# huang-yh/SelfOcc

Hardware: AMD Instinct MI355X
Metric: rendered rays/sec (6-cam 450x800, 128 samples/ray) (higher is better)
Workload: dtype f32; 1 GPU; BASELINE configs[1]: 6 cams x 450x800 rays, 128 samples/ray, volume 200x200x16; volume_channels=1, feat_storage=f32, preheat_steps=150

## Files before the change

### selfocc_amd/csrc/render_fwd.hip

```cpp
#include "so_device.h"
#include "sh_device.h"
#include "ray_device.h"

template <int NF, bool BF16>
int so_render_fwd_samples(const so_render_args &a, hipStream_t st);
template <int NB>
int so_render_sh_samples(const so_render_args &a, hipStream_t st);

namespace {

SO_DEVFN RayGeom so_pixel_ray(const so_render_args &a, int cam, int ix, int iy) {
    typedef const __attribute__((address_space(4))) float *so_const_fptr;
    const so_const_fptr M = (so_const_fptr)(a.img2lidar + cam * 16);
    float u = (float)ix * a.sx + a.ox;
    float v = (float)iy * a.sy + a.oy;
    RayGeom g;
    g.ox = M[3]; g.oy = M[7]; g.oz = M[11];
    float dx = (M[0] * u + M[1] * v) + M[2];
    float dy = (M[4] * u + M[5] * v) + M[6];
    float dz = (M[8] * u + M[9] * v) + M[10];
    g.dn = sqrtf((dx * dx + dy * dy) + dz * dz);
    g.dx = dx / g.dn; g.dy = dy / g.dn; g.dz = dz / g.dn;
    return g;
}
// ... 345 lines not shown
#pragma unroll
        for (int kk = 0; kk < 8; ++kk) {
            const int h = h0 + (kk >> 2), w = w0 + ((kk >> 1) & 1), d = d0 + (kk & 1);
            const bool in = ((unsigned)h < (unsigned)H) && ((unsigned)w < (unsigned)W) && ((unsigned)d < (unsigned)D);
            const int li = ((min(max(h, 0), H - 1) - hmin) * 4 + (min(max(w, 0), W - 1) - wmin)) * 4 +
                           (min(max(d, 0), D - 1) - dmin);
            const float wgt = in ? wk[kk] : 0.0f;
            const float4 *p = (const float4 *)(lds + li * ST);
#pragma unroll
            for (int q = 0; q < NF / 4; ++q) {
                const float4 t = p[q];
                so_fma4_bcast(f[4 * q + 0], f[4 * q + 1], f[4 * q + 2], f[4 * q + 3], t.x, t.y,
                              t.z, t.w, wgt);
            }
        }
    }
    __builtin_amdgcn_fence(__ATOMIC_RELEASE, "wavefront");
    __builtin_amdgcn_wave_barrier();
}

SO_DEVFN so_render_args so_reload_args() {
    typedef const __attribute__((address_space(4))) uint32_t *so_kernarg_ptr;
    so_kernarg_ptr ka = (so_kernarg_ptr)__builtin_amdgcn_kernarg_segment_ptr();
    asm volatile("" : "+s"(ka));
    so_render_args ac;
    static_assert(sizeof(ac) % 4 == 0, "so_render_args is dword-sized");
#pragma unroll
    for (unsigned k = 0; k < sizeof(ac) / 4; ++k) ((uint32_t *)&ac)[k] = ka[k];
    return ac;
}

template <int NF>
struct FastStep {
    float fh, fw, fd, fi;
    int h0, w0, d0;
    unsigned cell;
    bool all_interior;
    float v[8];
    unsigned code;
    bool boxed, pref;
    int hmin, wmin, dmin;
    so_f4v blk[NF >= 4 ? NF / 4 : 1];
};

template <int NF, bool BF16, bool STAGED = false, bool FACE_SAFE = false, class GeomFn>
SO_DEVFN void so_march_fast(const so_render_args &a, int ray, GeomFn geom, bool store = true,
                             float *lds = nullptr, int lane = 0, float *sem_lds = nullptr) {
    constexpr int NSEM = NF > 4 ? NF - 3 : 0;
    constexpr bool SEM_LDS = STAGED && NSEM >= 16;
    const RayGeom g = geom(a);
    const int H = a.map.h.tot_len, W = a.map.w.tot_len, D = a.map.d.tot_len;
    const int S = a.n_samples;
    float tnear, tfar;
    so_collide(a, g, tnear, tfar);
    const float dt = (tfar - tnear) / (float)S;
    const float inv_dn = 1.0f / g.dn;

    const AxisK kh = so_axis_affine(a.map.h), kw = so_axis_affine(a.map.w), kd = so_axis_affine(a.map.d);
    const float t_off = (a.sample_pos == SO_SAMPLE_AT_START) ? tnear : tnear + 0.5f * dt;
    const float Gdh = g.dy * kh.k1, Gdw = g.dx * kw.k1, Gdd = g.dz * kd.k1;
    const float G0h = fmaf(g.oy, kh.k1, kh.k0) + Gdh * t_off;
    const float G0w = fmaf(g.ox, kw.k1, kw.k0) + Gdw * t_off;
    const float G0d = fmaf(g.oz, kd.k1, kd.k0) + Gdd * t_off;
    const float s2 = so_inv_s(a) * 1.44269504088896341f;
    const float hdt = 0.5f * dt;
    const float hdt_s2 = hdt * s2;

    float T = 1.0f, acc = 0.0f, dsum = 0.0f;
    float rgb[3] = {0.0f, 0.0f, 0.0f};
    float sem[(NSEM > 0 && !SEM_LDS) ? NSEM : 1];
    if constexpr (SEM_LDS) {
#pragma unroll
        for (int k = 0; k < NSEM; ++k) sem_lds[k * 256] = 0.0f;
    } else {
#pragma unroll
        for (int k = 0; k < NSEM; ++k) sem[k] = 0.0f;
    }
    float best_w = -1.0f, best_t = 0.0f;
    const float *__restrict__ vol = a.sdf_vol;
    const __amdgpu_buffer_rsrc_t rs = so_make_rsrc(vol, (size_t)H * W * D * 4);
    const unsigned sD = (unsigned)D * 4u, sWD = (unsigned)W * D * 4u;
    const bool use_brick = a.sdf_brick != nullptr;
    const unsigned n_cells = (unsigned)(H * W * D);
    const __amdgpu_buffer_rsrc_t rb = so_make_rsrc(a.sdf_brick, use_brick ? (size_t)n_cells * 33 : 0);
    const unsigned lane_vox = (unsigned)(((lane >> 4) * W + ((lane >> 2) & 3)) * D + (lane & 3));
    const __amdgpu_buffer_rsrc_t rf = so_make_rsrc(a.feat_vol, NF > 0 ? (size_t)H * W * D * NF * (BF16 ? 2 : 4) : 0);
    constexpr bool CAN_SKIP = NF == 0;
    const bool use_skip = CAN_SKIP && use_brick && !(a.flags & SO_FLAG_NO_SKIP);
    const int rcode = use_skip ? max((int)ceilf(dt / so_skip_unit(a.aabb, S)), 1) : 0x7fffffff;
    const int maxdim = max(H, max(W, D));
    const float face_m = 3.0f * 1.1920929e-7f * (float)(1u << (32 - __builtin_clz((unsigned)maxdim)));

    constexpr bool FACE_LATE = FACE_SAFE && NF == 0;
    auto near_face = [&](float fh, float fw, float fd) __attribute__((always_inline)) {
        return fmaxf(fmaxf(fabsf(fh - 0.5f), fabsf(fw - 0.5f)), fabsf(fd - 0.5f)) > 0.5f - face_m;
    };
    auto canon_cell = [&](const int i) __attribute__((always_inline)) {
        if constexpr (NF < 8) {
            const float b0 = so_bin(i, S);
            const float t_start = b0 * tfar + (1.0f - b0) * tnear;
            float px, py, pz;
            if (a.sample_pos == SO_SAMPLE_AT_START) {
                px = g.ox + g.dx * t_start; py = g.oy + g.dy * t_start; pz = g.oz + g.dz * t_start;
            } else {
                const float b1 = so_bin(i + 1, S);
                const float tt = t_start + (b1 * tfar + (1.0f - b1) * tnear);
                px = g.ox + (g.dx * tt) / 2.0f; py = g.oy + (g.dy * tt) / 2.0f; pz = g.oz + (g.dz * tt) / 2.0f;
            }
            return so_locate(a.map, px, py, pz);
        } else {
            const so_render_args ac = so_reload_args();
            const RayGeom gc = geom(ac);
            float tn, tf;
            so_collide(ac, gc, tn, tf);
            const float t_start = so_edge(ac, ray, i, tn, tf);
            float px, py, pz;
            if (ac.sample_pos == SO_SAMPLE_AT_START) {
                px = gc.ox + gc.dx * t_start; py = gc.oy + gc.dy * t_start; pz = gc.oz + gc.dz * t_start;
            } else {
                const float tt = t_start + so_edge(ac, ray, i + 1, tn, tf);
                px = gc.ox + (gc.dx * tt) / 2.0f; py = gc.oy + (gc.dy * tt) / 2.0f; pz = gc.oz + (gc.dz * tt) / 2.0f;
            }
            return so_locate(ac.map, px, py, pz);
        }
    };

    constexpr bool PIPE = NF < 8;
    auto fetch = [&](const int i, FastStep<NF> &st) __attribute__((always_inline)) {
        st.fi = (float)i;
        const float step = st.fi * dt;
        const float gh = fmaf(Gdh, step, G0h), gw = fmaf(Gdw, step, G0w), gd = fmaf(Gdd, step, G0d);
        st.fh = __builtin_amdgcn_fractf(gh); st.fw = __builtin_amdgcn_fractf(gw); st.fd = __builtin_amdgcn_fractf(gd);
        int h0 = so_floor_i(gh), w0 = so_floor_i(gw), d0 = so_floor_i(gd);
        if constexpr (FACE_SAFE && !FACE_LATE) {
            if (__any(near_face(st.fh, st.fw, st.fd))) {
                if (near_face(st.fh, st.fw, st.fd)) {
                    const so_cell c = canon_cell(i);
                    h0 = c.h0; w0 = c.w0; d0 = c.d0;
                    st.fh = c.fh1; st.fw = c.fw1; st.fd = c.fd1;
                }
            }
        }
        st.h0 = h0; st.w0 = w0; st.d0 = d0;
        const bool interior = ((unsigned)h0 < (unsigned)(H - 1)) & ((unsigned)w0 < (unsigned)(W - 1)) &
                              ((unsigned)d0 < (unsigned)(D - 1));
        st.all_interior = so_all(interior);
        st.cell = so_cell_index(h0, w0, d0, W, D);
        st.code = 0u;
        if (st.all_interior) {
            if (use_brick) {
                const unsigned vo = st.cell * 32u;
                const so_f4v lo = so_bload4(rb, vo, 0u), hi = so_bload4(rb, vo + 16u, 0u);
                if constexpr (CAN_SKIP) {
                    if (use_skip) st.code = __builtin_amdgcn_raw_buffer_load_b8(rb, st.cell, n_cells * 32u, 0);
                }
                st.v[0] = lo.x; st.v[4] = lo.y; st.v[1] = lo.z; st.v[5] = lo.w;
                st.v[2] = hi.x; st.v[6] = hi.y; st.v[3] = hi.z; st.v[7] = hi.w;
            } else {
                const unsigned vo = st.cell * 4u;
                const so_f2v p00 = so_bload2(rs, vo, 0u), p01 = so_bload2(rs, vo, sD);
                const so_f2v p10 = so_bload2(rs, vo, sWD), p11 = so_bload2(rs, vo, sWD + sD);
                st.v[0] = p00.x; st.v[1] = p00.y; st.v[2] = p01.x; st.v[3] = p01.y;
                st.v[4] = p10.x; st.v[5] = p10.y; st.v[6] = p11.x; st.v[7] = p11.y;
            }
        } else {
            const int d0c = min(max(d0, 0), D - 2);
            const bool dlo_in = (unsigned)d0 < (unsigned)D, dhi_in = (unsigned)(d0 + 1) < (unsigned)D;
            const bool lo_first = (d0 == d0c), hi_first = (d0 + 1 == d0c);
#pragma unroll
            for (int q = 0; q < 4; ++q) {
                const int h = h0 + (q >> 1), w = w0 + (q & 1);
                const bool in = ((unsigned)h < (unsigned)H) && ((unsigned)w < (unsigned)W);
                const int hc = min(max(h, 0), H - 1), wc = min(max(w, 0), W - 1);
                const so_f2u pr = *(const so_f2u *)(vol + ((hc * W + wc) * D + d0c));
                const float lo = lo_first ? pr.x : pr.y, hi = hi_first ? pr.x : pr.y;
                st.v[2 * q] = (in && dlo_in) ? lo : 0.0f;
                st.v[2 * q + 1] = (in && dhi_in) ? hi : 0.0f;
            }
        }
        st.boxed = false; st.pref = false;
        if constexpr (STAGED) {
            st.boxed = so_stage_box(h0, w0, d0, H, W, D, st.hmin, st.wmin, st.dmin);
            if (PIPE && st.boxed && st.hmin + 3 < H && st.wmin + 3 < W && st.dmin + 3 < D) {
                const unsigned vo = ((unsigned)((st.hmin * W + st.wmin) * D + st.dmin) + lane_vox) * (NF * 4u);
#pragma unroll
                for (int q = 0; q < NF / 4; ++q) st.blk[q] = so_bload4(rf, vo + q * 16u, 0u);
                st.pref = true;
            }
        }
    };

    auto consume = [&](const int i, FastStep<NF> &st) __attribute__((always_inline)) {
        const float fi = st.fi;
        const float *v = st.v;
        float w, sdf = 0.0f, gvw = 0.0f, gvd = 0.0f, gvh = 0.0f;
        bool skip = false;
        if constexpr (CAN_SKIP) skip = so_all((int)st.code >= rcode);
        if (skip) {
            w = kAlphaFree * T;
            T = T * ((1.0f - kAlphaFree) + 1e-7f);
        } else {
            if constexpr (FACE_LATE) {
                if (__any(near_face(st.fh, st.fw, st.fd))) {
                    if (near_face(st.fh, st.fw, st.fd)) {
                        const so_cell c = canon_cell(i);
                        if (c.h0 != st.h0 || c.w0 != st.w0 || c.d0 != st.d0) {
                            so_gather_sdf(vol, H, W, D, c, st.v);
                            st.fh = c.fh1; st.fw = c.fw1; st.fd = c.fd1;
                            st.h0 = c.h0; st.w0 = c.w0; st.d0 = c.d0;
                        }
                    }
                }
            }
            const float fh = st.fh, fw = st.fw, fd = st.fd;
            const float dd0 = v[1] - v[0], dd1 = v[3] - v[2], dd2 = v[5] - v[4], dd3 = v[7] - v[6];
            const float c0 = fmaf(fd, dd0, v[0]), c1 = fmaf(fd, dd1, v[2]);
            const float c2 = fmaf(fd, dd2, v[4]), c3 = fmaf(fd, dd3, v[6]);
            const float dw0 = c1 - c0, dw1 = c3 - c2;
            const float b0 = fmaf(fw, dw0, c0), b1 = fmaf(fw, dw1, c2);
            const float dh0 = b1 - b0;
            sdf = fmaf(fh, dh0, b0);
            gvw = fmaf(fh, dw1 - dw0, dw0);
            const float e0 = fmaf(fw, dd1 - dd0, dd0), e1 = fmaf(fw, dd3 - dd2, dd2);
            gvd = fmaf(fh, e1 - e0, e0);
            gvh = dh0;

            const float cosv = fmaf(gvd, Gdd, fmaf(gvw, Gdw, gvh * Gdh));
            const float alpha = so_alpha_fast(sdf * s2, fminf(cosv, 0.0f) * hdt_s2);
            w = alpha * T;
            T = T * ((1.0f - alpha) + 1e-7f);
        }

        const float t_mid = fmaf(fi, dt, tnear + hdt);
        acc = acc + w;
        dsum = fmaf(w, t_mid, dsum);
        if (w > best_w) { best_w = w; best_t = t_mid; }

// ... 21 lines not shown
                else so_gather_feat<NF, BF16>(a.feat_vol, H, W, D, c, wk, f);
            }
#pragma unroll
            for (int k = 0; k < 3; ++k) {
                float col = fmaxf(fmaf(0.28209479177387814f, f[k], 0.5f), 0.0f);
                rgb[k] = fmaf(w, col, rgb[k]);
            }
            if constexpr (NSEM > 0) {
                float m = f[3];
#pragma unroll
                for (int k = 1; k < NSEM; ++k) m = fmaxf(m, f[3 + k]);
                float e[NSEM], den = 0.0f;
#pragma unroll
                for (int k = 0; k < NSEM; ++k) {
                    e[k] = so_fast_exp2((f[3 + k] - m) * 1.44269504088896341f);
                    den = den + e[k];
                }
                const float wd = w * so_fast_rcp(den);
                if constexpr (SEM_LDS) {
#pragma unroll
                    for (int k = 0; k < NSEM; ++k) sem_lds[k * 256] = fmaf(wd, e[k], sem_lds[k * 256]);
                } else {
#pragma unroll
                    for (int k = 0; k < NSEM; ++k) sem[k] = fmaf(wd, e[k], sem[k]);
                }
            }
        }
    };

    if constexpr (PIPE) {
        FastStep<NF> A, B;
        fetch(0, A);
        for (int i = 0;;) {
            if (i + 1 < S) fetch(i + 1, B);
            consume(i, A);
            if (++i >= S) break;
            if (so_all(T < 1e-10f)) break;
            if (i + 1 < S) fetch(i + 1, A);
            consume(i, B);
            if (++i >= S) break;
            if (so_all(T < 1e-10f)) break;
        }
    } else {
        for (int i = 0; i < S; ++i) {
            FastStep<NF> A;
            fetch(i, A);
            consume(i, A);
            if (so_all(T < 1e-10f)) break;
        }
    }

    const float eps32 = 1.1920928955078125e-07f;
    if (dt * inv_dn < eps32) best_t = tnear + hdt;
    if (!store) return;
    float depth = dsum * so_fast_rcp(acc + 1e-10f);
    if (a.flags & SO_FLAG_DEPTH_DIV_NORM) depth = depth * inv_dn;
    if (a.depth) a.depth[ray] = depth;
    if (a.acc) a.acc[ray] = acc;
    if (a.max_depth) a.max_depth[ray] = best_t * inv_dn;
    if (a.nears) a.nears[ray] = tnear;
    if (a.fars) a.fars[ray] = tfar;
    if constexpr (NF > 0) {
        if (a.rgb) {
#pragma unroll
            for (int k = 0; k < 3; ++k) {
                float bg = 0.0f;
                if (a.bkgd_mode == SO_BKGD_CONST) bg = a.bkgd[k];
                else if (a.bkgd_mode == SO_BKGD_PER_RAY) bg = a.bkgd_rays[3 * (size_t)ray + k];
                float r = rgb[k];
                if (a.bkgd_mode != SO_BKGD_NONE) r = r + bg * (1.0f - acc);
                if (a.flags & SO_FLAG_CLAMP_RGB) r = fminf(fmaxf(r, 0.0f), 1.0f);
                a.rgb[3 * (size_t)ray + k] = r;
            }
        }
        if constexpr (NSEM > 0) {
            if (a.sem) {
#pragma unroll
                for (int k = 0; k < NSEM; ++k) a.sem[(size_t)ray * NSEM + k] = SEM_LDS ? sem_lds[k * 256] : sem[k];
            }
        }
    }
}

struct AheadStep {
    float gh, gw, gd, fi;
    int h0, w0, d0;
    unsigned cell, code;
    bool all_interior;
};

template <bool FACE_SAFE, class GeomFn>
SO_DEVFN void so_march_fast_ahead(const so_render_args &a, int ray, GeomFn geom) {
    const int H = a.map.h.tot_len, W = a.map.w.tot_len, D = a.map.d.tot_len;
    const int S = a.n_samples;
    const RayGeom g = geom(a);
    float tnear, tfar;
    so_collide(a, g, tnear, tfar);
    const float dt = (tfar - tnear) / (float)S;
    const float inv_dn = 1.0f / g.dn;
    const AxisK kh = so_axis_affine(a.map.h), kw = so_axis_affine(a.map.w), kd = so_axis_affine(a.map.d);
    const float t_off = (a.sample_pos == SO_SAMPLE_AT_START) ? tnear : tnear + 0.5f * dt;
    const float Gdh = g.dy * kh.k1, Gdw = g.dx * kw.k1, Gdd = g.dz * kd.k1;
    const float G0h = fmaf(g.oy, kh.k1, kh.k0) + Gdh * t_off;
    const float G0w = fmaf(g.ox, kw.k1, kw.k0) + Gdw * t_off;
    const float G0d = fmaf(g.oz, kd.k1, kd.k0) + Gdd * t_off;
    const float s2 = so_inv_s(a) * 1.44269504088896341f;
    const float hdt = 0.5f * dt, hdt_s2 = hdt * s2;
    const float *__restrict__ vol = a.sdf_vol;
    const unsigned n_cells = (unsigned)(H * W * D);
    const __amdgpu_buffer_rsrc_t rb = so_make_rsrc(a.sdf_brick, (size_t)n_cells * 33);
    const __amdgpu_buffer_rsrc_t rs = so_make_rsrc(vol, (size_t)n_cells * 4);
    const int rcode = max((int)ceilf(dt / so_skip_unit(a.aabb, S)), 1);
    const int maxdim = max(H, max(W, D));
    const float face_m = 3.0f * 1.1920929e-7f * (float)(1u << (32 - __builtin_clz((unsigned)maxdim)));

    float T = 1.0f, acc = 0.0f, dsum = 0.0f, best_w = -1.0f, best_t = 0.0f;

    auto locate = [&](const int i, AheadStep &st) __attribute__((always_inline)) {
        st.fi = (float)i;
        const float step = st.fi * dt;
        const float gh = fmaf(Gdh, step, G0h), gw = fmaf(Gdw, step, G0w), gd = fmaf(Gdd, step, G0d);
        st.gh = gh; st.gw = gw; st.gd = gd;
        const int h0 = so_floor_i(gh), w0 = so_floor_i(gw), d0 = so_floor_i(gd);
        st.h0 = h0; st.w0 = w0; st.d0 = d0;
        st.all_interior = so_all3((unsigned)h0 < (unsigned)(H - 1), (unsigned)w0 < (unsigned)(W - 1),
                                  (unsigned)d0 < (unsigned)(D - 1));
        st.cell = so_cell_index(h0, w0, d0, W, D);
        st.code = 0u;
        if (st.all_interior) st.code = __builtin_amdgcn_raw_buffer_load_b8(rb, st.cell, n_cells * 32u, 0);
    };
    auto near_face = [&](float fh, float fw, float fd) __attribute__((always_inline)) {
        return fmaxf(fmaxf(fabsf(fh - 0.5f), fabsf(fw - 0.5f)), fabsf(fd - 0.5f)) > 0.5f - face_m;
    };
    auto canon_cell = [&](const int i) __attribute__((always_inline)) {
        const RayGeom gc = geom(so_reload_args());
        __builtin_amdgcn_sched_barrier(0);
        float px, py, pz;
        {
            const so_render_args ac = so_reload_args();
            const int n = ac.n_samples;
            const float b0 = so_bin(i, n);
            const float t_start = b0 * tfar + (1.0f - b0) * tnear;
            if (ac.sample_pos == SO_SAMPLE_AT_START) {
                px = gc.ox + gc.dx * t_start; py = gc.oy + gc.dy * t_start; pz = gc.oz + gc.dz * t_start;
            } else {
                const float b1 = so_bin(i + 1, n);
                const float tt = t_start + (b1 * tfar + (1.0f - b1) * tnear);
                px = gc.ox + (gc.dx * tt) / 2.0f; py = gc.oy + (gc.dy * tt) / 2.0f; pz = gc.oz + (gc.dz * tt) / 2.0f;
            }
        }
        __builtin_amdgcn_sched_barrier(0);
        float slope;
        const float gh = so_grid_coord(so_axis_m2g(so_reload_args().map.h, py, slope), so_reload_args().map.h.tot_len);
        __builtin_amdgcn_sched_barrier(0);
        const float gw = so_grid_coord(so_axis_m2g(so_reload_args().map.w, px, slope), so_reload_args().map.w.tot_len);
        __builtin_amdgcn_sched_barrier(0);
        const float gd = so_grid_coord(so_axis_m2g(so_reload_args().map.d, pz, slope), so_reload_args().map.d.tot_len);
        return so_cell_of(gh, gw, gd);
    };

    auto step = [&](const int i, AheadStep &cur, AheadStep &nxt) __attribute__((always_inline)) {
        const bool skip = cur.all_interior && so_all((int)cur.code >= rcode);
        if (i + 1 < S) locate(i + 1, nxt);
        float w;
        if (skip) {
            w = kAlphaFree * T;
            T = T * ((1.0f - kAlphaFree) + 1e-7f);
        } else {
            float fh = __builtin_amdgcn_fractf(cur.gh), fw = __builtin_amdgcn_fractf(cur.gw), fd = __builtin_amdgcn_fractf(cur.gd);
            so_f32x2 p0, p1, p2, p3;
            auto gather = [&](int h0, int w0, int d0) __attribute__((always_inline)) {
                float v[8];
                so_gather_sdf_buf(rs, H, W, D, h0, w0, d0, v);
                p0 = so_f32x2{v[0], v[4]}; p1 = so_f32x2{v[1], v[5]}; p2 = so_f32x2{v[2], v[6]}; p3 = so_f32x2{v[3], v[7]};
            };
            bool loaded = false;
            if constexpr (FACE_SAFE) {
                if (__any(near_face(fh, fw, fd))) {
                    int h0 = cur.h0, w0 = cur.w0, d0 = cur.d0;
                    bool moved = false;
                    if (near_face(fh, fw, fd)) {
                        const so_cell c = canon_cell(i);
                        if (c.h0 != h0 || c.w0 != w0 || c.d0 != d0) {
                            h0 = c.h0; w0 = c.w0; d0 = c.d0;
                            fh = c.fh1; fw = c.fw1; fd = c.fd1;
                            moved = true;
                        }
                    }
                    if (__any(moved)) { gather(h0, w0, d0); loaded = true; }
                }
            }
            if (!loaded) {
                if (cur.all_interior) {
                    {
                        const so_f4v lo = so_bload4(rb, cur.cell * 32u, 0u), hi = so_bload4(rb, cur.cell * 32u + 16u, 0u);
                        p0 = lo.xy; p1 = lo.zw; p2 = hi.xy; p3 = hi.zw;
                    }
                } else {
                    gather(cur.h0, cur.w0, cur.d0);
                }
            }
            float sdf, dh0, gvw, gvd;
            so_trilerp_fast_pk(p0, p1, p2, p3, fh, fw, fd, sdf, dh0, gvw, gvd);
            const float cosv = fmaf(gvd, Gdd, fmaf(gvw, Gdw, dh0 * Gdh));
            const float alpha = so_alpha_fast(sdf * s2, fminf(cosv, 0.0f) * hdt_s2);
            w = alpha * T;
            T = T * ((1.0f - alpha) + 1e-7f);
        }
        const float t_mid = fmaf(cur.fi, dt, tnear + hdt);
        acc = acc + w;
        dsum = fmaf(w, t_mid, dsum);
        if (w > best_w) { best_w = w; best_t = t_mid; }
    };

    {
        AheadStep A, B;
        locate(0, A);
        for (int i = 0;;) {
            step(i, A, B);
            if (++i >= S) break;
            if (so_all(T < 1e-10f)) break;
            step(i, B, A);
            if (++i >= S) break;
            if (so_all(T < 1e-10f)) break;
        }
    }

    const float eps32 = 1.1920928955078125e-07f;
    if (dt * inv_dn < eps32) best_t = tnear + hdt;
    float depth = dsum * so_fast_rcp(acc + 1e-10f);
    if (a.flags & SO_FLAG_DEPTH_DIV_NORM) depth = depth * inv_dn;
    if (a.depth) a.depth[ray] = depth;
    if (a.acc) a.acc[ray] = acc;
    if (a.max_depth) a.max_depth[ray] = best_t * inv_dn;
    if (a.nears) a.nears[ray] = tnear;
    if (a.fars) a.fars[ray] = tfar;
}

enum class March {
    Canonical,
    Fast,
    FastFaceSafe,
    Skip,
    SkipFaceSafe,
    CanonicalUpscale,
};
constexpr bool so_is_fast(March m) { return m == March::Fast || m == March::FastFaceSafe; }
constexpr bool so_is_skip(March m) { return m == March::Skip || m == March::SkipFaceSafe; }
constexpr bool so_face_safe(March m) { return m == March::FastFaceSafe || m == March::SkipFaceSafe; }
template <int NF, bool BF16>
constexpr bool so_is_staged(March m) { return so_is_fast(m) && !BF16 && NF >= 4; }

template <int NF, bool BF16, March MODE, class GeomFn>
SO_DEVFN void so_march(const so_render_args &a, int ray, GeomFn geom) {
    if constexpr (MODE == March::CanonicalUpscale) {
        so_march_exact<NF, BF16, SO_MAP_UPSCALE>(a, ray, geom(a));
    } else if constexpr (so_is_skip(MODE)) {
        static_assert(NF == 0, "skip marcher: SDF-only launches");
        so_march_fast_ahead<so_face_safe(MODE)>(a, ray, geom);
    } else if constexpr (so_is_fast(MODE)) {
        so_march_fast<NF, BF16, false, so_face_safe(MODE)>(a, ray, geom);
    } else {
        so_march_exact<NF, BF16>(a, ray, geom(a));
    }
}


__global__ __launch_bounds__(256) void sdf_brickify_kernel(const float *__restrict__ vol, float *__restrict__ brick,
                                                           int H, int W, int D, so_render_args a, int with_codes) {
    const int cell = blockIdx.x * blockDim.x + threadIdx.x;
    if (cell >= H * W * D) return;
    const int d = cell % D, w = (cell / D) % W, h = cell / (D * W);
    const int h1 = min(h + 1, H - 1), w1 = min(w + 1, W - 1), d1 = min(d + 1, D - 1);
    const float *r00 = vol + ((size_t)h * W + w) * D, *r01 = vol + ((size_t)h * W + w1) * D;
    const float *r10 = vol + ((size_t)h1 * W + w) * D, *r11 = vol + ((size_t)h1 * W + w1) * D;
    const float v0 = r00[d], v1 = r00[d1], v2 = r01[d], v3 = r01[d1];
    const float v4 = r10[d], v5 = r10[d1], v6 = r11[d], v7 = r11[d1];
    float4 *o = (float4 *)(brick + (size_t)cell * 8);
    o[0] = make_float4(v0, v4, v1, v5);
    o[1] = make_float4(v2, v6, v3, v7);
    uint8_t *codes = (uint8_t *)(brick + (size_t)H * W * D * 8);
    unsigned code = 0u;
    if (with_codes) {
        const float m = fminf(fminf(fminf(v0, v1), fminf(v2, v3)), fminf(fminf(v4, v5), fminf(v6, v7)));
        const float gd = fmaxf(fmaxf(fabsf(v1 - v0), fabsf(v3 - v2)), fmaxf(fabsf(v5 - v4), fabsf(v7 - v6))) *
                         (a.map.d.size0 / a.map.d.range0);
        const float gw = fmaxf(fmaxf(fabsf(v2 - v0), fabsf(v3 - v1)), fmaxf(fabsf(v6 - v4), fabsf(v7 - v5))) *
                         (a.map.w.size0 / a.map.w.range0);
        const float gh = fmaxf(fmaxf(fabsf(v4 - v0), fabsf(v5 - v1)), fmaxf(fabsf(v6 - v2), fabsf(v7 - v3))) *
                         (a.map.h.size0 / a.map.h.range0);
        const float G = sqrtf((gd * gd + gw * gw) + gh * gh) * 1.001f + 1e-20f;
        const float slack = m - kSkipArg / so_inv_s(a);
        if (slack > 0.0f && so_inv_s(a) > 0.0f) {
            const float allow = 2.0f * slack / G / so_skip_unit(a.aabb, a.n_samples);
            code = (unsigned)fminf(floorf(allow * 0.999f), 255.0f);
        }
    }
    codes[cell] = (uint8_t)code;
}

struct TilePixel { int cam, ix, iy, wave, lane; };
SO_DEVFN TilePixel so_tile_pixel(int tiles_x, int tiles_y) {
    const int b = blockIdx.x;
    const int cam = b / (tiles_x * tiles_y);
    const int tb = b - cam * tiles_x * tiles_y;
    const int ty = tb / tiles_x, tx = tb - ty * tiles_x;
    const int wave = threadIdx.x >> 6, lane = threadIdx.x & 63;
    return {cam, tx * 16 + (wave & 1) * 8 + (lane & 7), ty * 16 + (wave >> 1) * 8 + (lane >> 3), wave, lane};
}

template <int NF, bool BF16, March MODE>
__global__ __launch_bounds__(256, (NF >= 8 ? 2 : 1)) void render_fwd_explicit(so_render_args a) {
    int ray = blockIdx.x * blockDim.x + threadIdx.x;
    if (ray >= a.n_rays) return;
    auto geom = [&](const so_render_args &a) __attribute__((always_inline)) { return so_explicit_ray(a, ray); };
    so_march<NF, BF16, MODE>(a, ray, geom);
}

template <int NF, bool BF16, March MODE>
SO_DEVFN void pixgrid_body(const so_render_args &a, int tiles_x, int tiles_y) {
    const TilePixel p = so_tile_pixel(tiles_x, tiles_y);
    const int cam = p.cam, wave = p.wave, lane = p.lane;
    int ix = p.ix, iy = p.iy;
    if constexpr (so_is_staged<NF, BF16>(MODE)) {
        __shared__ __attribute__((aligned(16))) float s_stage[4 * StageGeom<NF>::kWaveDwords];
        const bool real = (ix < a.nx) && (iy < a.ny);
        ix = min(ix, a.nx - 1); iy = min(iy, a.ny - 1);
        int ray = (cam * a.ny + iy) * a.nx + ix;
        auto geom = [&](const so_render_args &a) __attribute__((always_inline)) { return so_pixel_ray(a, cam, ix, iy); };
        constexpr int NSEM_LDS = NF - 3 >= 16 ? NF - 3 : 0;
        __shared__ float s_sem[NSEM_LDS > 0 ? NSEM_LDS * 256 : 1];
        so_march_fast<NF, BF16, true, so_face_safe(MODE)>(a, ray, geom, real, s_stage + wave * StageGeom<NF>::kWaveDwords, lane,
                                                          s_sem + threadIdx.x);
    } else {
        if (ix >= a.nx || iy >= a.ny) return;
        int ray = (cam * a.ny + iy) * a.nx + ix;
        auto geom = [&](const so_render_args &a) __attribute__((always_inline)) { return so_pixel_ray(a, cam, ix, iy); };
        so_march<NF, BF16, MODE>(a, ray, geom);
    }
}

template <int NF, bool BF16, March MODE>
__global__ __launch_bounds__(256, (NF >= 8 ? 2 : 1)) void render_fwd_pixgrid(so_render_args a, int tiles_x, int tiles_y) {
    pixgrid_body<NF, BF16, MODE>(a, tiles_x, tiles_y);
}
template <>
__global__ __launch_bounds__(256, 1) __attribute__((amdgpu_num_sgpr(80))) void render_fwd_pixgrid<0, false, March::Skip>(
    so_render_args a, int tiles_x, int tiles_y) {
    pixgrid_body<0, false, March::Skip>(a, tiles_x, tiles_y);
}
template <>
__global__ __launch_bounds__(256, 1) __attribute__((amdgpu_num_sgpr(80))) void render_fwd_pixgrid<0, false, March::SkipFaceSafe>(
    so_render_args a, int tiles_x, int tiles_y) {
    pixgrid_body<0, false, March::SkipFaceSafe>(a, tiles_x, tiles_y);
}

template <int NF, bool BF16, March MODE>
int launch_fwd(const so_render_args &a, hipStream_t st) {
    if (a.ray_mode == SO_RAYS_EXPLICIT) {
        int blocks = (a.n_rays + 255) / 256;
        hipLaunchKernelGGL((render_fwd_explicit<NF, BF16, MODE>), dim3(blocks), dim3(256), 0, st, a);
    } else {
        int tiles_x = (a.nx + 15) / 16, tiles_y = (a.ny + 15) / 16;
        int blocks = tiles_x * tiles_y * a.n_cams;
        hipLaunchKernelGGL((render_fwd_pixgrid<NF, BF16, MODE>), dim3(blocks), dim3(256), 0, st, a, tiles_x, tiles_y);
    }
    return so_launch_status();
}

template <int NF, bool BF16>
int dispatch_ps(const so_render_args &a, hipStream_t st) {
    bool per_sample = a.weights || a.ts || a.deltas || a.sdf || a.grad;
    if (per_sample) return so_render_fwd_samples<NF, BF16>(a, st);
    if (a.map.kind == SO_MAP_UPSCALE) {
        if constexpr (NF == 24 && BF16) {
            SO_REQUIRE(false, "the 'linear_upscale' mapping is built for n_rgb + n_sem = 0, 3, 8 and float32 24 (got bfloat16 24)");
        } else {
            return launch_fwd<NF, BF16, March::CanonicalUpscale>(a, st);
        }
    }
    bool fast = !(a.flags & SO_FLAG_EXACT) && a.jitter_mode == SO_JITTER_NONE && a.map.kind == SO_MAP_LINEAR &&
                a.map.h.size1 == 0.0f && a.map.w.size1 == 0.0f && a.map.d.size1 == 0.0f &&
                (long long)a.map.h.tot_len * a.map.w.tot_len < (1 << 24) && a.map.d.tot_len < (1 << 24);
    if (fast) {
        if (a.sdf_brick) {
            const int cells = a.map.h.tot_len * a.map.w.tot_len * a.map.d.tot_len;
            const int with_codes = (NF == 0 && !(a.flags & SO_FLAG_NO_SKIP)) ? 1 : 0;
            hipLaunchKernelGGL(sdf_brickify_kernel, dim3((cells + 255) / 256), dim3(256), 0, st, a.sdf_vol, a.sdf_brick,
                               a.map.h.tot_len, a.map.w.tot_len, a.map.d.tot_len, a, with_codes);
        }
        if constexpr (NF == 0) {
            if (a.sdf_brick && !(a.flags & (SO_FLAG_NO_SKIP | SO_FLAG_NO_AHEAD)))
                return (a.flags & SO_FLAG_NO_FACE_SAFE) ? launch_fwd<0, false, March::Skip>(a, st) : launch_fwd<0, false, March::SkipFaceSafe>(a, st);
        }
        if (!(a.flags & SO_FLAG_NO_FACE_SAFE)) return launch_fwd<NF, BF16, March::FastFaceSafe>(a, st);
        return launch_fwd<NF, BF16, March::Fast>(a, st);
    }
    return launch_fwd<NF, BF16, March::Canonical>(a, st);
}

template <int NB, int MK>
__global__ __launch_bounds__(256) void render_sh_explicit(so_render_args a) {
    const int ray = blockIdx.x * blockDim.x + threadIdx.x;
    if (ray >= a.n_rays) return;
    so_march_exact<so_sh_stride(NB), false, MK, NB>(a, ray, so_explicit_ray(a, ray));
}

template <int NB, int MK>
__global__ __launch_bounds__(256) void render_sh_pixgrid(so_render_args a, int tiles_x, int tiles_y) {
    const int b = blockIdx.x;
    const int cam = b / (tiles_x * tiles_y);
    const int tb = b - cam * tiles_x * tiles_y;
    const int ty = tb / tiles_x, tx = tb - ty * tiles_x;
    const int wave = threadIdx.x >> 6, lane = threadIdx.x & 63;
    const int ix = tx * 16 + (wave & 1) * 8 + (lane & 7);
    const int iy = ty * 16 + (wave >> 1) * 8 + (lane >> 3);
    if (ix >= a.nx || iy >= a.ny) return;
    const int ray = (cam * a.ny + iy) * a.nx + ix;
    so_march_exact<so_sh_stride(NB), false, MK, NB>(a, ray, so_pixel_ray(a, cam, ix, iy));
}

template <int NB, int MK>
int launch_sh(const so_render_args &a, hipStream_t st) {
    if (a.ray_mode == SO_RAYS_EXPLICIT) {
        hipLaunchKernelGGL((render_sh_explicit<NB, MK>), dim3((a.n_rays + 255) / 256), dim3(256), 0, st, a);
    } else {
        const int tiles_x = (a.nx + 15) / 16, tiles_y = (a.ny + 15) / 16;
        hipLaunchKernelGGL((render_sh_pixgrid<NB, MK>), dim3(tiles_x * tiles_y * a.n_cams), dim3(256), 0, st, a, tiles_x, tiles_y);
    }
    return so_launch_status();
}

template <int NB>
int dispatch_sh(const so_render_args &a, hipStream_t st) {
    if (a.weights || a.ts || a.deltas || a.sdf || a.grad) return so_render_sh_samples<NB>(a, st);
    return a.map.kind == SO_MAP_UPSCALE ? launch_sh<NB, SO_MAP_UPSCALE>(a, st) : launch_sh<NB, SO_MAP_LINEAR>(a, st);
}

}

int so_validate_mapping(const so_mapping &m) {
    SO_REQUIRE(m.kind == SO_MAP_LINEAR || m.kind == SO_MAP_UPSCALE, "mapping: unknown kind %d (0 = linear, 1 = linear_upscale)",
               (int)m.kind);
    const so_axis *ax[3] = {&m.h, &m.w, &m.d};
    const so_upscale_axis *ux[3] = {&m.uh, &m.uw, &m.ud};
    for (int i = 0; i < 3; ++i) {
        SO_REQUIRE(ax[i]->tot_len >= 2, "mapping axis %d: tot_len must be >= 2", i);
        SO_REQUIRE(ax[i]->size0 > 0 && ax[i]->range0 > 0, "mapping axis %d: size0/range0 must be > 0", i);
        if (m.kind == SO_MAP_LINEAR) {
            SO_REQUIRE(ax[i]->size1 == 0 || ax[i]->range1 > 0, "mapping axis %d: range1 must be > 0", i);
        } else {
            SO_REQUIRE(ax[i]->size1 >= 1, "linear_upscale axis %d: outer cells must be >= 1 (got %g)", i, (double)ax[i]->size1);
            SO_REQUIRE(ux[i]->unit > 0 && __builtin_isfinite(ux[i]->unit), "linear_upscale axis %d: unit must be > 0 (got %g)", i,
                       (double)ux[i]->unit);
            SO_REQUIRE(ux[i]->inc > 0 && __builtin_isfinite(ux[i]->inc),
                       "linear_upscale axis %d: increase unit must be > 0 (got %g): the outer range must exceed outer * unit",
                       i, (double)ux[i]->inc);
        }
    }
    return 0;
}

namespace {
template <int MK>
__global__ __launch_bounds__(256) void meter2grid_kernel(so_mapping m, const float *__restrict__ xyz, int n, int normalize,
                                                         float *__restrict__ hwd) {
    const int i = blockIdx.x * blockDim.x + threadIdx.x;
    if (i >= n) return;
    float gh, gw, gd, sh, sw, sd;
    so_m2g<MK>(m, xyz[3 * (size_t)i], xyz[3 * (size_t)i + 1], xyz[3 * (size_t)i + 2], gh, gw, gd, sh, sw, sd);
    if (normalize) {
        gh = gh / (float)(m.h.tot_len - 1); gw = gw / (float)(m.w.tot_len - 1); gd = gd / (float)(m.d.tot_len - 1);
// ... 84 lines not shown
```

### selfocc_amd/render.py

```python
import os
from dataclasses import dataclass, field
from typing import Optional

import torch

from . import abi, sh
from ._lib import lib, check, ptr, current_stream


@dataclass
class SDFVolume:
    mapping: object
    sdf: torch.Tensor
    feat: Optional[torch.Tensor] = None
    n_rgb: int = 0
    n_sem: int = 0
    sh_deg: int = 0
    sh_act: str = 'relu'

    @staticmethod
    def feat_width(n_rgb, n_sem, sh_deg=0):
        if n_rgb + n_sem == 0:
            return 0
        if sh_deg > 0:
# ... 116 lines not shown
        a.feat_vol = ptr(vol.feat)
        a.feat_dtype = abi.DTYPE_F32 if vol.feat.dtype == torch.float32 else abi.DTYPE_BF16
        a.feat_stride = vol.feat.shape[3]
    N = rays.n_rays
    a.n_rays = N
    keep = [vol, rays, t_rand, bkgd_rays]
    if rays.pixel_grid:
        a.ray_mode = abi.RAYS_PIXEL_GRID
        a.img2lidar = ptr(_c(rays.img2lidar))
        a.n_cams, a.nx, a.ny = rays.img2lidar.shape[0], rays.nx, rays.ny
        a.sx, a.sy, a.ox, a.oy = rays.sx, rays.sy, rays.ox, rays.oy
    else:
        a.ray_mode = abi.RAYS_EXPLICIT
        a.origins, a.dirs = ptr(_c(rays.origins)), ptr(_c(rays.dirs))
        a.dir_norm = ptr(None if rays.dir_norm is None else _c(rays.dir_norm))
    for i in range(6):
        a.aabb[i] = float(cfg.aabb[i])
    a.near_plane = cfg.near_plane
    a.n_samples = S = cfg.n_samples
    a.sample_pos = cfg.sample_pos
    a.jitter_mode = cfg.jitter_mode
    if cfg.jitter_mode != abi.JITTER_NONE:
        exp = (N,) if cfg.jitter_mode == abi.JITTER_SINGLE else (N, S + 1)
        assert t_rand is not None and tuple(t_rand.shape) == exp, f"t_rand must be {exp}"
        a.t_rand = ptr(_c(t_rand))
    a.inv_s = float(cfg.inv_s)
    if cfg.inv_s_dev is not None:
        t = cfg.inv_s_dev
        assert t.dtype == torch.float32 and t.numel() == 1 and t.device == dev, "inv_s_dev: one float32 on the volume's device"
        a.inv_s_dev = ptr(t)
        keep.append(t)
    a.bkgd_mode = cfg.bkgd_mode
    for i in range(3):
        a.bkgd[i] = float(cfg.bkgd[i])
    if cfg.bkgd_mode == abi.BKGD_PER_RAY:
        assert bkgd_rays is not None and tuple(bkgd_rays.shape) == (N, 3)
        a.bkgd_rays = ptr(_c(bkgd_rays))
    a.flags = (abi.FLAG_DEPTH_DIV_NORM if cfg.depth_div_norm else 0) | (abi.FLAG_CLAMP_RGB if cfg.clamp_rgb else 0) | \
        (abi.FLAG_EXACT if cfg.exact else 0) | (0 if cfg.skip else abi.FLAG_NO_SKIP) | \
        (0 if cfg.face_safe else abi.FLAG_NO_FACE_SAFE) | (0 if cfg.ahead else abi.FLAG_NO_AHEAD) | \
        (abi.FLAG_RAY_PER_LANE if cfg.ray_per_lane else 0)

    f32 = dict(dtype=torch.float32, device=dev)
    out = outputs if outputs is not None else {}
    def alloc(name, *shape):
        if name not in out:
            out[name] = torch.empty(*shape, **f32)
        return ptr(out[name])
    a.depth, a.acc = alloc('depth', N), alloc('acc', N)
    a.max_depth, a.nears, a.fars = alloc('max_depth', N), alloc('nears', N), alloc('fars', N)
    if vol.n_rgb == 3:
        a.rgb = alloc('rgb', N, 3)
    if vol.n_sem > 0:
        a.sem = alloc('sem', N, vol.n_sem)
    if per_sample:
        a.weights, a.ts, a.deltas = alloc('weights', N, S), alloc('ts', N, S), alloc('deltas', N, S)
        if want_grad_samples:
            a.sdf, a.grad = alloc('sdf', N, S), alloc('grad', N, S, 3)
    keep.append(out)
    return a, out, keep


def render_rays(vol: SDFVolume, rays: RaySet, cfg: RenderConfig, *, per_sample=False,
                want_grad_samples=False, t_rand=None, bkgd_rays=None, outputs=None):
    if not vol.sdf.is_cuda:
        raise RuntimeError("selfocc_amd.render_rays needs CUDA(HIP) tensors: there is no CPU fallback")
    a, out, _keep = marshal_render_args(vol, rays, cfg, per_sample=per_sample,
                                        want_grad_samples=want_grad_samples, t_rand=t_rand,
                                        bkgd_rays=bkgd_rays, outputs=outputs)
    if cfg.brick and not cfg.exact and a.map.kind == abi.MAP_LINEAR and rays.n_rays * cfg.n_samples >= 16 * vol.sdf.numel():
        a.sdf_brick = ptr(_brick_workspace(vol.sdf))
    check(lib().selfocc_render_fwd(a, current_stream(vol.sdf.device)), "selfocc_render_fwd")
    return out


_BRICK_WS = {}


def _brick_workspace(sdf):
    key = (sdf.device, torch.cuda.current_stream(sdf.device).cuda_stream, tuple(sdf.shape))
    ws = _BRICK_WS.get(key)
    if ws is None:
        n = sdf.numel()
        ws = _BRICK_WS[key] = torch.empty((n * 33 + 15) // 16 * 16, dtype=torch.uint8, device=sdf.device)
    return ws


def _scatter_workspace(device, nbytes):
    return torch.empty(nbytes, dtype=torch.uint8, device=device)


class _RenderFunction(torch.autograd.Function):

    @staticmethod
    def forward(ctx, sdf_vol, feat_vol, inv_s, mapping, n_rgb, n_sem, rays, cfg, t_rand, bkgd_rays, want_grad_samples,
                sh_deg=0, sh_act='relu'):
        vol = SDFVolume(mapping, sdf_vol, feat_vol, n_rgb, n_sem, sh_deg, sh_act)
        cfg_run = RenderConfig(**{**cfg.__dict__, 'inv_s_dev': inv_s.detach().reshape(1).float().contiguous()})
        out = render_rays(vol, rays, cfg_run, per_sample=True, want_grad_samples=want_grad_samples,
                          t_rand=t_rand, bkgd_rays=bkgd_rays)
        ctx.has = (feat_vol is not None, t_rand is not None, bkgd_rays is not None)
        ctx.save_for_backward(*[t for t in (sdf_vol, feat_vol, t_rand, bkgd_rays, cfg_run.inv_s_dev) if t is not None])
        ctx.meta = (mapping, n_rgb, n_sem, sh_deg, sh_act)
        ctx.rays, ctx.cfg = rays, RenderConfig(**{**cfg_run.__dict__, 'inv_s_dev': None})
        ctx.inv_s_shape = inv_s.shape
        ctx.keys = ['depth', 'acc'] + (['rgb'] if n_rgb else []) + (['sem'] if n_sem else []) + ['weights'] + \
            (['sdf', 'grad'] if want_grad_samples else [])
        ctx.nondiff_keys = ['ts', 'deltas', 'max_depth', 'nears', 'fars']
        nd = tuple(out[k] for k in ctx.nondiff_keys)
        ctx.mark_non_differentiable(*nd)
        return tuple(out[k] for k in ctx.keys) + nd

    @staticmethod
    def backward(ctx, *grads):
        saved = list(ctx.saved_tensors)
        sdf_vol = saved.pop(0)
        feat_vol = saved.pop(0) if ctx.has[0] else None
        t_rand = saved.pop(0) if ctx.has[1] else None
        bkgd_rays = saved.pop(0) if ctx.has[2] else None
        inv_s_dev = saved.pop(0)
        vol = SDFVolume(ctx.meta[0], sdf_vol, feat_vol, *ctx.meta[1:])
        rays, cfg = ctx.rays, RenderConfig(**{**ctx.cfg.__dict__, 'inv_s_dev': inv_s_dev})
        gmap = {k: g for k, g in zip(ctx.keys, grads)}
        a, _out, _keep = marshal_render_args(vol, rays, cfg, per_sample=False, t_rand=t_rand,
                                             bkgd_rays=bkgd_rays, outputs={})
        ba = abi.SoRenderBwdArgs()
        ba.fwd = a
        hold = []
        def gp(name):
            g = gmap.get(name)
            if g is None:
                return None
            g = g.contiguous().float()
            hold.append(g)
            return ptr(g)
        ba.g_depth, ba.g_acc, ba.g_rgb, ba.g_sem = gp('depth'), gp('acc'), gp('rgb'), gp('sem')
        ba.g_weights, ba.g_sdf, ba.g_grad = gp('weights'), gp('sdf'), gp('grad')
        g_sdf_vol = torch.zeros_like(vol.sdf)
        ba.g_sdf_vol = ptr(g_sdf_vol)
        g_feat = None
        if vol.feat is not None and ctx.needs_input_grad[1]:
            g_feat = torch.zeros(vol.feat.shape, dtype=torch.float32, device=vol.feat.device)
            ba.g_feat_vol = ptr(g_feat)
        g_inv_s = torch.zeros(1, device=vol.sdf.device)
        ba.g_inv_s = ptr(g_inv_s)
        mode = cfg.bwd_scatter if cfg.bwd_scatter != 'auto' else os.environ.get('SELFOCC_RB_SCATTER', 'auto')
        if mode == 'binned' or (mode == 'auto' and rays.n_rays * cfg.n_samples >= (1 << 19)):
            need = int(lib().selfocc_render_bwd_ws_bytes(ba))
            if need > 0:
                ws = _scatter_workspace(vol.sdf.device, need)
                ba.scatter_ws, ba.scatter_ws_bytes = ptr(ws), ws.numel()
                hold.append(ws)
            elif mode == 'binned':
                raise RuntimeError("bwd_scatter='binned': the volume / launch is outside the binned scatter's range")
        check(lib().selfocc_render_bwd(ba, current_stream(vol.sdf.device)), "selfocc_render_bwd")
        if g_feat is not None and vol.feat.dtype != torch.float32:
            g_feat = g_feat.to(vol.feat.dtype)
        return (g_sdf_vol, g_feat, g_inv_s.reshape(ctx.inv_s_shape), None, None, None, None, None, None, None, None, None, None)


def render_rays_autograd(vol: SDFVolume, inv_s: torch.Tensor, rays: RaySet, cfg: RenderConfig, *,
                         want_grad_samples=True, t_rand=None, bkgd_rays=None):
    res = _RenderFunction.apply(vol.sdf, vol.feat, inv_s, vol.mapping, vol.n_rgb, vol.n_sem, rays, cfg,
                                t_rand, bkgd_rays, want_grad_samples, vol.sh_deg, vol.sh_act)
    keys = ['depth', 'acc'] + (['rgb'] if vol.n_rgb else []) + (['sem'] if vol.n_sem else []) + ['weights'] + \
        (['sdf', 'grad'] if want_grad_samples else []) + ['ts', 'deltas', 'max_depth', 'nears', 'fars']
    return dict(zip(keys, res))
# ... 1 lines not shown
```

Before: 6.552 billion rays/s.

## Halve brick layout, add free-space run loop, sure-interior range, and 2D brickify

The brick workspace shrinks from 8 floats per cell to 4. The upper half of each cell's corners is now read from the neighbouring d-row offset, which cuts brick memory traffic and footprint. The ahead march gains a precomputed range of sample indices known to be interior, so per-step bounds checks can be skipped. It also gains a tight 'run' loop that advances through free-space steps with a constant alpha while every lane's skip code allows it. The brickify kernel is relaid out as a 2D grid over (h,w) with d-threads and packs skip codes four at a time via DPP. The interior-range probe only scans a few samples at each end, so the adjacent-row brick read assumes that layout is valid at volume edges.

```diff
diff --git a/selfocc_amd/csrc/render_fwd.hip b/selfocc_amd/csrc/render_fwd.hip
--- a/selfocc_amd/csrc/render_fwd.hip
+++ b/selfocc_amd/csrc/render_fwd.hip
@@ -451,7 +451,7 @@
     const unsigned sD = (unsigned)D * 4u, sWD = (unsigned)W * D * 4u;
     const bool use_brick = a.sdf_brick != nullptr;
     const unsigned n_cells = (unsigned)(H * W * D);
-    const __amdgpu_buffer_rsrc_t rb = so_make_rsrc(a.sdf_brick, use_brick ? (size_t)n_cells * 33 : 0);
+    const __amdgpu_buffer_rsrc_t rb = so_make_rsrc(a.sdf_brick, use_brick ? (size_t)n_cells * 17 : 0);
     const unsigned lane_vox = (unsigned)(((lane >> 4) * W + ((lane >> 2) & 3)) * D + (lane & 3));
     const __amdgpu_buffer_rsrc_t rf = so_make_rsrc(a.feat_vol, NF > 0 ? (size_t)H * W * D * NF * (BF16 ? 2 : 4) : 0);
     constexpr bool CAN_SKIP = NF == 0;
@@ -518,10 +518,10 @@
         st.code = 0u;
         if (st.all_interior) {
             if (use_brick) {
-                const unsigned vo = st.cell * 32u;
-                const so_f4v lo = so_bload4(rb, vo, 0u), hi = so_bload4(rb, vo + 16u, 0u);
+                const unsigned vo = st.cell * 16u;
+                const so_f4v lo = so_bload4(rb, vo, 0u), hi = so_bload4(rb, vo, (unsigned)D * 16u);
                 if constexpr (CAN_SKIP) {
-                    if (use_skip) st.code = __builtin_amdgcn_raw_buffer_load_b8(rb, st.cell, n_cells * 32u, 0);
+                    if (use_skip) st.code = __builtin_amdgcn_raw_buffer_load_b8(rb, st.cell, n_cells * 16u, 0);
                 }
                 st.v[0] = lo.x; st.v[4] = lo.y; st.v[1] = lo.z; st.v[5] = lo.w;
                 st.v[2] = hi.x; st.v[6] = hi.y; st.v[3] = hi.z; st.v[7] = hi.w;
@@ -709,6 +709,9 @@
     }
 }
 
+constexpr int kRunExitFreeSteps = 60000;
+constexpr int kSureScan = 8;
+
 struct AheadStep {
     float gh, gw, gd, fi;
     int h0, w0, d0;
@@ -735,7 +738,7 @@
     const float hdt = 0.5f * dt, hdt_s2 = hdt * s2;
     const float *__restrict__ vol = a.sdf_vol;
     const unsigned n_cells = (unsigned)(H * W * D);
-    const __amdgpu_buffer_rsrc_t rb = so_make_rsrc(a.sdf_brick, (size_t)n_cells * 33);
+    const __amdgpu_buffer_rsrc_t rb = so_make_rsrc(a.sdf_brick, (size_t)n_cells * 17);
     const __amdgpu_buffer_rsrc_t rs = so_make_rsrc(vol, (size_t)n_cells * 4);
     const int rcode = max((int)ceilf(dt / so_skip_unit(a.aabb, S)), 1);
     const int maxdim = max(H, max(W, D));
@@ -743,18 +746,44 @@
 
     float T = 1.0f, acc = 0.0f, dsum = 0.0f, best_w = -1.0f, best_t = 0.0f;
 
-    auto locate = [&](const int i, AheadStep &st) __attribute__((always_inline)) {
+    auto place = [&](const int i, AheadStep &st) __attribute__((always_inline)) {
         st.fi = (float)i;
         const float step = st.fi * dt;
         const float gh = fmaf(Gdh, step, G0h), gw = fmaf(Gdw, step, G0w), gd = fmaf(Gdd, step, G0d);
         st.gh = gh; st.gw = gw; st.gd = gd;
         const int h0 = so_floor_i(gh), w0 = so_floor_i(gw), d0 = so_floor_i(gd);
         st.h0 = h0; st.w0 = w0; st.d0 = d0;
-        st.all_interior = so_all3((unsigned)h0 < (unsigned)(H - 1), (unsigned)w0 < (unsigned)(W - 1),
-                                  (unsigned)d0 < (unsigned)(D - 1));
         st.cell = so_cell_index(h0, w0, d0, W, D);
+    };
+    auto interior = [&](const AheadStep &st) __attribute__((always_inline)) {
+        return so_all3((unsigned)st.h0 < (unsigned)(H - 1), (unsigned)st.w0 < (unsigned)(W - 1), (unsigned)st.d0 < (unsigned)(D - 1));
+    };
+    int i_lo = S, i_hi = -1;
+    {
+        AheadStep p;
+        const int n = min(kSureScan, S);
+#pragma nounroll
+        for (int k = 0; k < n; ++k) {
+            place(k, p);
+            if (interior(p)) { i_lo = k; break; }
+        }
+        if (i_lo < S) {
+#pragma nounroll
+            for (int k = S - 1; k >= S - n && k >= i_lo; --k) {
+                place(k, p);
+                if (interior(p)) { i_hi = k; break; }
+            }
+        }
+        if (i_hi < 0) i_lo = S;
+    }
+    auto sure = [&](const int i) __attribute__((always_inline)) { return i >= i_lo && i <= i_hi; };
+
+    auto locate = [&](const int i, AheadStep &st) __attribute__((always_inline)) {
+        place(i, st);
+        st.all_interior = true;
+        if (!sure(i)) st.all_interior = interior(st);
         st.code = 0u;
-        if (st.all_interior) st.code = __builtin_amdgcn_raw_buffer_load_b8(rb, st.cell, n_cells * 32u, 0);
+        if (st.all_interior) st.code = __builtin_amdgcn_raw_buffer_load_b8(rb, st.cell, n_cells * 16u, 0);
     };
     auto near_face = [&](float fh, float fw, float fd) __attribute__((always_inline)) {
         return fmaxf(fmaxf(fabsf(fh - 0.5f), fabsf(fw - 0.5f)), fabsf(fd - 0.5f)) > 0.5f - face_m;
@@ -820,7 +849,7 @@
             if (!loaded) {
                 if (cur.all_interior) {
                     {
-                        const so_f4v lo = so_bload4(rb, cur.cell * 32u, 0u), hi = so_bload4(rb, cur.cell * 32u + 16u, 0u);
+                        const so_f4v lo = so_bload4(rb, cur.cell * 16u, 0u), hi = so_bload4(rb, cur.cell * 16u, (unsigned)D * 16u);
                         p0 = lo.xy; p1 = lo.zw; p2 = hi.xy; p3 = hi.zw;
                     }
                 } else {
@@ -838,18 +867,45 @@
         acc = acc + w;
         dsum = fmaf(w, t_mid, dsum);
         if (w > best_w) { best_w = w; best_t = t_mid; }
+        return skip;
+    };
+
+    auto run = [&](int &i, AheadStep &st) __attribute__((always_inline)) {
+        if (i < i_lo || i >= i_hi) return false;
+        auto free_step = [&]() __attribute__((always_inline)) {
+            const float t_mid = fmaf(st.fi, dt, tnear + hdt);
+            ++i;
+            place(i, st);
+            st.all_interior = true;
+            st.code = __builtin_amdgcn_raw_buffer_load_b8(rb, st.cell, n_cells * 16u, 0);
+            const float w = kAlphaFree * T;
+            T = T * ((1.0f - kAlphaFree) + 1e-7f);
+            acc = acc + w;
+            dsum = fmaf(w, t_mid, dsum);
+        };
+        if (S <= kRunExitFreeSteps && !so_all(T < 2e-10f)) {
+            while (i < i_hi && so_all((int)st.code >= rcode)) free_step();
+        } else {
+            while (i < i_hi && so_all((int)st.code >= rcode)) {
+                free_step();
+                if (so_all(T < 1e-10f)) return true;
+            }
+        }
+        return false;
     };
 
     {
         AheadStep A, B;
         locate(0, A);
         for (int i = 0;;) {
-            step(i, A, B);
+            const bool sa = step(i, A, B);
             if (++i >= S) break;
             if (so_all(T < 1e-10f)) break;
-            step(i, B, A);
+            if (sa && run(i, B)) break;
+            const bool sb = step(i, B, A);
             if (++i >= S) break;
             if (so_all(T < 1e-10f)) break;
+            if (sb && run(i, A)) break;
         }
     }
 
@@ -895,35 +951,44 @@
 
 __global__ __launch_bounds__(256) void sdf_brickify_kernel(const float *__restrict__ vol, float *__restrict__ brick,
                                                            int H, int W, int D, so_render_args a, int with_codes) {
-    const int cell = blockIdx.x * blockDim.x + threadIdx.x;
-    if (cell >= H * W * D) return;
-    const int d = cell % D, w = (cell / D) % W, h = cell / (D * W);
-    const int h1 = min(h + 1, H - 1), w1 = min(w + 1, W - 1), d1 = min(d + 1, D - 1);
-    const float *r00 = vol + ((size_t)h * W + w) * D, *r01 = vol + ((size_t)h * W + w1) * D;
-    const float *r10 = vol + ((size_t)h1 * W + w) * D, *r11 = vol + ((size_t)h1 * W + w1) * D;
-    const float v0 = r00[d], v1 = r00[d1], v2 = r01[d], v3 = r01[d1];
-    const float v4 = r10[d], v5 = r10[d1], v6 = r11[d], v7 = r11[d1];
-    float4 *o = (float4 *)(brick + (size_t)cell * 8);
-    o[0] = make_float4(v0, v4, v1, v5);
-    o[1] = make_float4(v2, v6, v3, v7);
-    uint8_t *codes = (uint8_t *)(brick + (size_t)H * W * D * 8);
-    unsigned code = 0u;
-    if (with_codes) {
-        const float m = fminf(fminf(fminf(v0, v1), fminf(v2, v3)), fminf(fminf(v4, v5), fminf(v6, v7)));
-        const float gd = fmaxf(fmaxf(fabsf(v1 - v0), fabsf(v3 - v2)), fmaxf(fabsf(v5 - v4), fabsf(v7 - v6))) *
-                         (a.map.d.size0 / a.map.d.range0);
-        const float gw = fmaxf(fmaxf(fabsf(v2 - v0), fabsf(v3 - v1)), fmaxf(fabsf(v6 - v4), fabsf(v7 - v5))) *
-                         (a.map.w.size0 / a.map.w.range0);
-        const float gh = fmaxf(fmaxf(fabsf(v4 - v0), fabsf(v5 - v1)), fmaxf(fabsf(v6 - v2), fabsf(v7 - v3))) *
-                         (a.map.h.size0 / a.map.h.range0);
-        const float G = sqrtf((gd * gd + gw * gw) + gh * gh) * 1.001f + 1e-20f;
-        const float slack = m - kSkipArg / so_inv_s(a);
-        if (slack > 0.0f && so_inv_s(a) > 0.0f) {
-            const float allow = 2.0f * slack / G / so_skip_unit(a.aabb, a.n_samples);
-            code = (unsigned)fminf(floorf(allow * 0.999f), 255.0f);
-        }
-    }
-    codes[cell] = (uint8_t)code;
+    const int h = blockIdx.x, h1 = min(h + 1, H - 1);
+    const size_t n_cells = (size_t)H * W * D;
+    uint8_t *codes = (uint8_t *)(brick + n_cells * 4);
+    const bool quads = (D & 3) == 0 && (blockDim.x & 3) == 0;
+    const float kd = a.map.d.size0 / a.map.d.range0, kw = a.map.w.size0 / a.map.w.range0, kh = a.map.h.size0 / a.map.h.range0;
+    for (int w = blockIdx.y * blockDim.y + threadIdx.y; w < W; w += gridDim.y * blockDim.y) {
+        const int w1 = min(w + 1, W - 1);
+        const float *r00 = vol + ((size_t)h * W + w) * D, *r01 = vol + ((size_t)h * W + w1) * D;
+        const float *r10 = vol + ((size_t)h1 * W + w) * D, *r11 = vol + ((size_t)h1 * W + w1) * D;
+        for (int d = threadIdx.x; d < D; d += blockDim.x) {
+            const int d1 = min(d + 1, D - 1);
+            const float v0 = r00[d], v1 = r00[d1], v2 = r01[d], v3 = r01[d1];
+            const float v4 = r10[d], v5 = r10[d1], v6 = r11[d], v7 = r11[d1];
+            const size_t cell = ((size_t)h * W + w) * D + d;
+            ((float4 *)brick)[cell] = make_float4(v0, v4, v1, v5);
+            unsigned code = 0u;
+            if (with_codes) {
+                const float m = fminf(fminf(fminf(v0, v1), fminf(v2, v3)), fminf(fminf(v4, v5), fminf(v6, v7)));
+                const float gd = fmaxf(fmaxf(fabsf(v1 - v0), fabsf(v3 - v2)), fmaxf(fabsf(v5 - v4), fabsf(v7 - v6))) * kd;
+                const float gw = fmaxf(fmaxf(fabsf(v2 - v0), fabsf(v3 - v1)), fmaxf(fabsf(v6 - v4), fabsf(v7 - v5))) * kw;
+                const float gh = fmaxf(fmaxf(fabsf(v4 - v0), fabsf(v5 - v1)), fmaxf(fabsf(v6 - v2), fabsf(v7 - v3))) * kh;
+                const float G = sqrtf((gd * gd + gw * gw) + gh * gh) * 1.001f + 1e-20f;
+                const float slack = m - kSkipArg / so_inv_s(a);
+                if (slack > 0.0f && so_inv_s(a) > 0.0f) {
+                    const float allow = 2.0f * slack / G / so_skip_unit(a.aabb, a.n_samples);
+                    code = (unsigned)fminf(floorf(allow * 0.999f), 255.0f);
+                }
+            }
+            if (quads) {
+                const unsigned c1 = (unsigned)__builtin_amdgcn_update_dpp(0, (int)code, 0x55, 0xf, 0xf, false);
+                const unsigned c2 = (unsigned)__builtin_amdgcn_update_dpp(0, (int)code, 0xaa, 0xf, 0xf, false);
+                const unsigned c3 = (unsigned)__builtin_amdgcn_update_dpp(0, (int)code, 0xff, 0xf, 0xf, false);
+                if ((d & 3) == 0) *(unsigned *)(codes + cell) = code | (c1 << 8) | (c2 << 16) | (c3 << 24);
+            } else {
+                codes[cell] = (uint8_t)code;
+            }
+        }
+    }
 }
 
 struct TilePixel { int cam, ix, iy, wave, lane; };
@@ -1011,10 +1076,13 @@
                 (long long)a.map.h.tot_len * a.map.w.tot_len < (1 << 24) && a.map.d.tot_len < (1 << 24);
     if (fast) {
         if (a.sdf_brick) {
-            const int cells = a.map.h.tot_len * a.map.w.tot_len * a.map.d.tot_len;
             const int with_codes = (NF == 0 && !(a.flags & SO_FLAG_NO_SKIP)) ? 1 : 0;
-            hipLaunchKernelGGL(sdf_brickify_kernel, dim3((cells + 255) / 256), dim3(256), 0, st, a.sdf_vol, a.sdf_brick,
-                               a.map.h.tot_len, a.map.w.tot_len, a.map.d.tot_len, a, with_codes);
+            const int H = a.map.h.tot_len, W = a.map.w.tot_len, D = a.map.d.tot_len;
+            int qx = 1;
+            while (qx < D && qx < 256) qx *= 2;
+            const int wy = 256 / qx;
+            hipLaunchKernelGGL(sdf_brickify_kernel, dim3(H, min((W + wy - 1) / wy, 65535)), dim3(qx, wy), 0, st, a.sdf_vol, a.sdf_brick,
+                               H, W, D, a, with_codes);
         }
         if constexpr (NF == 0) {
             if (a.sdf_brick && !(a.flags & (SO_FLAG_NO_SKIP | SO_FLAG_NO_AHEAD)))
diff --git a/selfocc_amd/render.py b/selfocc_amd/render.py
--- a/selfocc_amd/render.py
+++ b/selfocc_amd/render.py
@@ -222,7 +222,7 @@
     ws = _BRICK_WS.get(key)
     if ws is None:
         n = sdf.numel()
-        ws = _BRICK_WS[key] = torch.empty((n * 33 + 15) // 16 * 16, dtype=torch.uint8, device=sdf.device)
+        ws = _BRICK_WS[key] = torch.empty((n * 17 + 15) // 16 * 16, dtype=torch.uint8, device=sdf.device)
     return ws
 
 
```

Measured after the change: 6.811 billion rays/s, median of 6. 1.04x the previous value.
